# kthohr/mcmc

Measured on AMD Instinct MI355X. Metric: leapfrog-steps/sec (chains*dims*steps/s), HMC d=128 correlated Gaussian, 65536 chains, higher is better.
Workload: dtype f64

## Files before the change

include/mi_mcmc_engine/det_math.hpp:

```cpp
#pragma once

#include <hip/hip_runtime.h>
#include <stdint.h>

#define MI_HD __host__ __device__ __forceinline__

#if defined(__HIP_DEVICE_COMPILE__)
#define MI_NO_DS_MERGE __attribute__((target("no-load-store-opt")))
#else
#define MI_NO_DS_MERGE
#endif

namespace mi {

#ifndef MI_KC_MODE
#define MI_KC_MODE 1
#endif
#if defined(__HIP_DEVICE_COMPILE__) && MI_KC_MODE == 1
__device__ __forceinline__ double mi_kc(double c) { asm volatile("" : "+s"(c)); return c; }
#define MI_KC(c) ::mi::mi_kc(c)
#define MI_KCD(c, dep) ::mi::mi_kc(c)
#elif defined(__HIP_DEVICE_COMPILE__) && MI_KC_MODE == 2
template <uint64_t BITS>
__device__ __forceinline__ double mi_kc()
{
    uint32_t lo, hi;
    asm volatile("s_mov_b32 %0, %2\n\ts_mov_b32 %1, %3" : "=s"(lo), "=s"(hi) : "n"((uint32_t)BITS), "n"((uint32_t)(BITS >> 32)));
    return __builtin_bit_cast(double, ((uint64_t)hi << 32) | (uint64_t)lo);
}
template <uint64_t BITS>
__device__ __forceinline__ double mi_kcd(double dep)
{
    uint32_t lo, hi;
    asm volatile("s_mov_b32 %0, %2\n\ts_mov_b32 %1, %3" : "=s"(lo), "=s"(hi) : "n"((uint32_t)BITS), "n"((uint32_t)(BITS >> 32)), "v"(dep));
    return __builtin_bit_cast(double, ((uint64_t)hi << 32) | (uint64_t)lo);
}
#define MI_KC(c) (::mi::mi_kc<__builtin_bit_cast(uint64_t, (double)(c))>())
#define MI_KCD(c, dep) (::mi::mi_kcd<__builtin_bit_cast(uint64_t, (double)(c))>(dep))
#else
#define MI_KC(c) (c)
#define MI_KCD(c, dep) (c)
#endif


MI_HD uint64_t d2u(double x) { return __builtin_bit_cast(uint64_t, x); }
MI_HD double u2d(uint64_t u) { return __builtin_bit_cast(double, u); }
MI_HD double pow2i(int k) { return u2d((uint64_t)(k + 1023) << 52); }
MI_HD double dfma(double a, double b, double c) { return __builtin_fma(a, b, c); }
MI_HD bool is_finite(double x) { return (d2u(x) & 0x7ff0000000000000ULL) != 0x7ff0000000000000ULL; }

constexpr double LN2_HI = 0x1.62e42fee00000p-1;
constexpr double LN2_LO = 0x1.a39ef35793c76p-33;
constexpr double INV_LN2 = 0x1.71547652b82fep+0;
constexpr double PI_4 = 0x1.921fb54442d18p-1;
constexpr double INF = __builtin_huge_val();

MI_HD double det_exp(double x)
{
    if (x != x) return x;
    if (x > 709.782712893384) return INF;
    if (x < -745.2) return 0.0;
    const double kf = __builtin_rint(x * INV_LN2);
    const int k = (int)kf;
    double r = dfma(-kf, LN2_HI, x);
    r = dfma(-kf, LN2_LO, r);
    double p = MI_KCD(1.0 / 87178291200.0, r);
    p = dfma(p, r, MI_KCD(1.0 / 6227020800.0, p));
    p = dfma(p, r, MI_KCD(1.0 / 479001600.0, p));
    p = dfma(p, r, MI_KCD(1.0 / 39916800.0, p));
    p = dfma(p, r, MI_KCD(1.0 / 3628800.0, p));
    p = dfma(p, r, MI_KCD(1.0 / 362880.0, p));
    p = dfma(p, r, MI_KCD(1.0 / 40320.0, p));
    p = dfma(p, r, MI_KCD(1.0 / 5040.0, p));
    p = dfma(p, r, MI_KCD(1.0 / 720.0, p));
    p = dfma(p, r, MI_KCD(1.0 / 120.0, p));
    p = dfma(p, r, MI_KCD(1.0 / 24.0, p));
    p = dfma(p, r, MI_KCD(1.0 / 6.0, p));
    p = dfma(p, r, 0.5);
    p = dfma(p, r, 1.0);
    p = dfma(p, r, 1.0);
    const int k1 = k / 2, k2 = k - k1;
    return (p * pow2i(k1)) * pow2i(k2);
}

MI_HD double det_log(double x)
{
    if (x != x) return x;
    if (x < 0.0) return __builtin_nan("");
    if (x == 0.0) return -INF;
    if (x == INF) return x;
    int e = 0;
    uint64_t u = d2u(x);
    if ((u >> 52) == 0) { x = x * 0x1p54; u = d2u(x); e = -54; }
    e += (int)(u >> 52) - 1023;
    u = (u & 0x000fffffffffffffULL) | 0x3ff0000000000000ULL;
    double m = u2d(u);
    if (m > 0x1.6a09e667f3bcdp+0) { m = m * 0.5; e += 1; }
    const double f = m - 1.0;
    const double s = f / (2.0 + f);
    const double z = s * s;
    double p = MI_KCD(1.0 / 23.0, z);
    p = dfma(p, z, MI_KCD(1.0 / 21.0, p));
    p = dfma(p, z, MI_KCD(1.0 / 19.0, p));
    p = dfma(p, z, MI_KCD(1.0 / 17.0, p));
    p = dfma(p, z, MI_KCD(1.0 / 15.0, p));
    p = dfma(p, z, MI_KCD(1.0 / 13.0, p));
    p = dfma(p, z, MI_KCD(1.0 / 11.0, p));
    p = dfma(p, z, MI_KCD(1.0 / 9.0, p));
    p = dfma(p, z, MI_KCD(1.0 / 7.0, p));
    p = dfma(p, z, MI_KCD(1.0 / 5.0, p));
    p = dfma(p, z, MI_KCD(1.0 / 3.0, p));
    p = dfma(p, z, 1.0);
    const double lm = (2.0 * s) * p;
    const double ef = (double)e;
    return dfma(ef, LN2_HI, dfma(ef, LN2_LO, lm));
}

MI_HD double det_pow(double x, double y) { return det_exp(y * det_log(x)); }

MI_HD double norm_ppf(double p)
{
    if (p != p) return p;
    if (p <= 0.0) return -INF;
    if (p >= 1.0) return INF;
    const double q = p - 0.5;
    if (__builtin_fabs(q) <= 0.425) {
        const double r = 0.180625 - q * q;
        const double num = (((((((2.5090809287301226727e+3 * r + 3.3430575583588128105e+4) * r + 6.7265770927008700853e+4) * r + 4.5921953931549871457e+4) * r +
                               1.3731693765509461125e+4) * r + 1.9715909503065514427e+3) * r + 1.3314166789178437745e+2) * r + 3.3871328727963666080e+0) * q;
        const double den = (((((((5.2264952788528545610e+3 * r + 2.8729085735721942674e+4) * r + 3.9307895800092710610e+4) * r + 2.1213794301586595867e+4) * r +
                               5.3941960214247511077e+3) * r + 6.8718700749205790830e+2) * r + 4.2313330701600911252e+1) * r + 1.0);
        return num / den;
    }
    double r = __builtin_sqrt(-det_log(q <= 0.0 ? p : 1.0 - p));
    double num, den;
    if (r <= 5.0) {
        r = r - 1.6;
        num = (((((((7.74545014278341407640e-4 * r + 2.27238449892691845833e-2) * r + 2.41780725177450611770e-1) * r + 1.27045825245236838258e+0) * r +
                  3.64784832476320460504e+0) * r + 5.76949722146069140550e+0) * r + 4.63033784615654529590e+0) * r + 1.42343711074968357734e+0);
        den = (((((((1.05075007164441684324e-9 * r + 5.47593808499534494600e-4) * r + 1.51986665636164571966e-2) * r + 1.48103976427480074590e-1) * r +
                  6.89767334985100004550e-1) * r + 1.67638483018380384940e+0) * r + 2.05319162663775882187e+0) * r + 1.0);
    } else {
        r = r - 5.0;
        num = (((((((2.01033439929228813265e-7 * r + 2.71155556874348757815e-5) * r + 1.24266094738807843860e-3) * r + 2.65321895265761230930e-2) * r +
                  2.96560571828504891230e-1) * r + 1.78482653991729133580e+0) * r + 5.46378491116411436990e+0) * r + 6.65790464350110377720e+0);
        den = (((((((2.04426310338993978564e-15 * r + 1.42151175831644588870e-7) * r + 1.84631831751005468180e-5) * r + 7.86869131145613259100e-4) * r +
                  1.48753612908506148525e-2) * r + 1.36929880922735805310e-1) * r + 5.99832206555887937690e-1) * r + 1.0);
    }
    const double x = num / den;
    return q < 0.0 ? -x : x;
}

MI_HD void sincos_kernel(double a, double& s, double& c)
{
    const double z = a * a;
    double ps = MI_KCD(-1.0 / 121645100408832000.0, z);
    ps = dfma(ps, z, MI_KCD(1.0 / 355687428096000.0, ps));
    ps = dfma(ps, z, MI_KCD(-1.0 / 1307674368000.0, ps));
    ps = dfma(ps, z, MI_KCD(1.0 / 6227020800.0, ps));
    ps = dfma(ps, z, MI_KCD(-1.0 / 39916800.0, ps));
    ps = dfma(ps, z, MI_KCD(1.0 / 362880.0, ps));
    ps = dfma(ps, z, MI_KCD(-1.0 / 5040.0, ps));
    ps = dfma(ps, z, MI_KCD(1.0 / 120.0, ps));
    ps = dfma(ps, z, MI_KCD(-1.0 / 6.0, ps));
    ps = dfma(ps, z, 1.0);
    s = a * ps;
    double pc = MI_KCD(1.0 / 6402373705728000.0, z);
    pc = dfma(pc, z, MI_KCD(-1.0 / 20922789888000.0, pc));
    pc = dfma(pc, z, MI_KCD(1.0 / 87178291200.0, pc));
    pc = dfma(pc, z, MI_KCD(-1.0 / 479001600.0, pc));
    pc = dfma(pc, z, MI_KCD(1.0 / 3628800.0, pc));
    pc = dfma(pc, z, MI_KCD(-1.0 / 40320.0, pc));
    pc = dfma(pc, z, MI_KCD(1.0 / 720.0, pc));
    pc = dfma(pc, z, MI_KCD(-1.0 / 24.0, pc));
    pc = dfma(pc, z, 0.5);
    c = dfma(-pc, z, 1.0);
}

MI_HD void det_sincos2pi(double u, double& sn, double& cs)
{
    const double v = u * 8.0;
    const double qf = __builtin_floor(v);
    const int q = (int)qf & 7;
    double t = v - qf;
    if (q & 1) t = 1.0 - t;
    double s, c;
    sincos_kernel(t * PI_4, s, c);
    const bool swap = ((q + 1) & 2) != 0;
    const double cc = swap ? s : c;
    const double ss = swap ? c : s;
    const bool neg_c = (q >= 2) && (q <= 5);
    const bool neg_s = (q >= 4);
    cs = neg_c ? -cc : cc;
    sn = neg_s ? -ss : ss;
}

MI_HD double softplus(double eta)
{
    if (eta > 0.0) return eta + det_log(1.0 + det_exp(-eta));
    return det_log(1.0 + det_exp(eta));
}
MI_HD double sigmoid(double eta)
{
    if (eta >= 0.0) return 1.0 / (1.0 + det_exp(-eta));
    const double e = det_exp(eta);
    return e / (1.0 + e);
}

struct u32x4 { uint32_t x, y, z, w; };

MI_HD uint32_t mulhi32(uint32_t a, uint32_t b) { return (uint32_t)(((uint64_t)a * b) >> 32); }

MI_HD u32x4 philox4x32_10(u32x4 c, uint32_t k0, uint32_t k1)
{
#pragma unroll
    for (int r = 0; r < 10; ++r) {
        const uint64_t p0 = (uint64_t)0xD2511F53u * c.x, p1 = (uint64_t)0xCD9E8D57u * c.z;
        c = u32x4{(uint32_t)(p1 >> 32) ^ c.y ^ k0, (uint32_t)p1, (uint32_t)(p0 >> 32) ^ c.w ^ k1, (uint32_t)p0};
        k0 += 0x9E3779B9u;
        k1 += 0xBB67AE85u;
    }
    return c;
}

MI_HD double u01(uint32_t lo, uint32_t hi)
{
    const uint64_t k = (((uint64_t)hi << 32) | lo) >> 12;
    return (double)(2 * k + 1) * 0x1p-53;
}

enum : uint32_t { STREAM_NORMAL = 0u, STREAM_UNIFORM = 1u, STREAM_INIT = 2u,
                  STREAM_DE_INIT = 3u, STREAM_DE = 4u,
                  STREAM_AEES_NORMAL = 5u, STREAM_AEES = 6u,
                  STREAM_BRIDGE = 7u,
                  STREAM_PREDICT = 8u };

MI_HD u32x4 rng_block(uint64_t seed, uint64_t chain, uint32_t draw, uint32_t slot, uint32_t stream)
{
    const u32x4 c{(uint32_t)chain, draw, slot, stream | ((uint32_t)(chain >> 32) << 8)};
    return philox4x32_10(c, (uint32_t)seed, (uint32_t)(seed >> 32));
}

MI_HD double rng_uniform(uint64_t seed, uint64_t chain, uint32_t draw, uint32_t slot)
{
    const u32x4 w = rng_block(seed, chain, draw, slot, STREAM_UNIFORM);
    return u01(w.x, w.y);
}

MI_HD void rng_normal_pair_core(uint64_t seed, uint64_t chain, uint32_t draw, uint32_t slot, uint32_t stream, double& z0, double& z1)
{
    const u32x4 w = rng_block(seed, chain, draw, slot, stream);
    const double u1 = u01(w.x, w.y);
    const double u2 = u01(w.z, w.w);
    const double r = __builtin_sqrt(-2.0 * det_log(u1));
    double s, c;
    det_sincos2pi(u2, s, c);
    z0 = r * c;
    z1 = r * s;
}
#ifdef MI_RNG_NOINLINE
__attribute__((noinline))
#endif
MI_HD void rng_normal_pair(uint64_t seed, uint64_t chain, uint32_t draw, uint32_t slot, uint32_t stream,
                           double& z0, double& z1)
{
#if defined(__HIP_DEVICE_COMPILE__)
    asm volatile("" : "+v"(slot));
#endif
    rng_normal_pair_core(seed, chain, draw, slot, stream, z0, z1);
}

typedef double rng_double4 __attribute__((ext_vector_type(4)));
__device__ __attribute__((noinline)) inline rng_double4 rng_normal_two_pairs(uint64_t seed, uint64_t chain, uint32_t draw, uint32_t slot_a,
                                                                             uint32_t slot_b, uint32_t stream)
{
#if defined(__HIP_DEVICE_COMPILE__)
    asm volatile("" : "+v"(slot_a), "+v"(slot_b));
#endif
    double a0, a1, b0, b1;
    rng_normal_pair_core(seed, chain, draw, slot_a, stream, a0, a1);
    rng_normal_pair_core(seed, chain, draw, slot_b, stream, b0, b1);
    return rng_double4{a0, a1, b0, b1};
}
typedef double rng_double8 __attribute__((ext_vector_type(8)));
__device__ __attribute__((noinline)) inline rng_double8 rng_normal_four_pairs(uint64_t seed, uint64_t chain, uint32_t draw, uint32_t slot_a,
                                                                              uint32_t slot_step, uint32_t stream)
{
#if defined(__HIP_DEVICE_COMPILE__)
    asm volatile("" : "+v"(slot_a));
#endif
    double z[8];
#pragma unroll
    for (int k = 0; k < 4; ++k) rng_normal_pair_core(seed, chain, draw, slot_a + (uint32_t)k * slot_step, stream, z[2 * k], z[2 * k + 1]);
    return rng_double8{z[0], z[1], z[2], z[3], z[4], z[5], z[6], z[7]};
}

MI_HD void rng_normal_pair_at(uint64_t seed, uint64_t chain, uint32_t draw, uint32_t base, uint32_t j, uint32_t stream,
                              double& z0, double& z1)
{
#if defined(__HIP_DEVICE_COMPILE__)
    asm volatile("" : "+v"(j));
#endif
    rng_normal_pair(seed, chain, draw, base + j, stream, z0, z1);
}


}
```

include/mi_mcmc_engine/hmc_dense.hpp:

```cpp
#pragma once

#include "det_math.hpp"

#ifndef MI_HMC_RNG_STAGED
#define MI_HMC_RNG_STAGED 0
#endif

#ifndef MI_HMC_RNG_PAIRS
#define MI_HMC_RNG_PAIRS 1
#endif

#ifndef MI_HMC_WPB
#define MI_HMC_WPB 8
#endif

namespace mi {

typedef double double4_t __attribute__((ext_vector_type(4)));

struct HmcParams {
    const double* P;
    uint32_t d;
    uint64_t C;
    uint64_t chain0;
    double* theta;
    double* wsave;
    int vals_bound;
    uint32_t draw0;
    const double* Minv;
    const double* Lchol;
    double* draws;
    uint64_t* n_accept;
    uint64_t* n_leap;
    uint64_t seed;
    uint32_t n_burnin, n_keep, n_leap_steps;
    double eps;
    const int* btype;
    const double* lb;
    const double* ub;
    const double* m_sqrt;
    const double* m_inv;
    uint32_t ablate;
    uint32_t stagger;
    uint32_t m_per_chain;
    uint32_t* nf_flag;
    uint32_t sep_target;
};

template <int NS>
__device__ __forceinline__ double dot4(const double (&x)[NS], const double (&y)[NS])
{
    double q = 0.0;
#pragma unroll
    for (int s = 0; s < NS; ++s) q = dfma(x[s], y[s], q);
    q = q + __shfl_xor(q, 32);
    q = q + __shfl_xor(q, 16);
    return q;
}

template <int NS>
__device__ __forceinline__ void dense_product_poison(const double (&x)[NS], double (&y)[NS], int j, uint32_t d)
{
    int nloc = 0;
#pragma unroll
    for (int s = 0; s < NS; ++s) nloc += is_finite(x[s]) ? 0 : 1;
    int n = nloc + __shfl_xor(nloc, 16);
    n = n + __shfl_xor(n, 32);
    if (__ballot(n != 0) == 0ull) return;
#pragma unroll
    for (int s = 0; s < NS; ++s) {
        const int others = n - (is_finite(x[s]) ? 0 : 1);
        if (others > 0 && (uint32_t)(4 * s + j) < d) y[s] = __builtin_nan("");
    }
}

template <int NT>
__device__ __forceinline__ void matvec_mfma(const double* __restrict__ afrag, const double (&th)[4 * NT],
                                            double (&w)[4 * NT])
{
    constexpr int NS = 4 * NT;
    double4_t acc[NT];
    double a_cur[NT], a_nxt[NT];
    typedef const double __attribute__((address_space(3)))* lds_cptr;
    lds_cptr lo = (lds_cptr)afrag;
    uint32_t hi_off = (uint32_t)(uintptr_t)lo + (NT > 4 ? 4u * NS * 64u * 8u : 0u);
    if constexpr (NT > 4) asm volatile("" : "+v"(hi_off));
    lds_cptr hi = (lds_cptr)(uintptr_t)hi_off;
    auto frag = [&](int t, int s) __attribute__((always_inline)) -> double {
        return (NT > 4 && t >= 4) ? hi[((t - 4) * NS + s) * 64] : lo[(t * NS + s) * 64];
    };
#pragma unroll
    for (int t = 0; t < NT; ++t) {
        acc[t] = double4_t{0.0, 0.0, 0.0, 0.0};
        a_cur[t] = frag(t, 0);
    }
#pragma unroll
    for (int s = 0; s < NS; ++s) {
        if (s + 1 < NS) {
#pragma unroll
            for (int t = 0; t < NT; ++t) a_nxt[t] = frag(t, s + 1);
        }
        __builtin_amdgcn_sched_barrier(0);
#pragma unroll
        for (int t = 0; t < NT; ++t)
            acc[t] = __builtin_amdgcn_mfma_f64_16x16x4f64(a_cur[t], th[s], acc[t], 0, 0, 0);
        __builtin_amdgcn_sched_barrier(0);
#pragma unroll
        for (int t = 0; t < NT; ++t) a_cur[t] = a_nxt[t];
    }
#pragma unroll
    for (int t = 0; t < NT; ++t) {
        w[4 * t + 0] = acc[t][0];
        w[4 * t + 1] = acc[t][1];
        w[4 * t + 2] = acc[t][2];
        w[4 * t + 3] = acc[t][3];
    }
}

template <int NT>
__device__ __forceinline__ void stage_precision(const double* __restrict__ P, uint32_t d, double* lds)
{
    constexpr int NS = 4 * NT;
    const int lane = threadIdx.x & 63, wave = threadIdx.x >> 6, nw = blockDim.x >> 6;
    for (int f = wave; f < NT * NS; f += nw) {
        const int t = f / NS, s = f % NS;
        const uint32_t row = 16 * t + (lane & 15), col = 4 * s + (lane >> 4);
        lds[f * 64 + lane] = (row < d && col < d) ? P[(size_t)row * d + col] : 0.0;
    }
    __syncthreads();
}


template <int NT>
__device__ __forceinline__ void matvec_mfma_g(const double* __restrict__ gfrag, const double (&th)[4 * NT], double (&w)[4 * NT])
{
    constexpr int NS = 4 * NT;
    constexpr int PD = 3;
    uint32_t b_lo = (uint32_t)__builtin_amdgcn_readfirstlane((int)(uint32_t)(uintptr_t)gfrag);
    uint32_t b_hi = (uint32_t)__builtin_amdgcn_readfirstlane((int)(uint32_t)((uintptr_t)gfrag >> 32));
    asm volatile("" : "+s"(b_lo), "+s"(b_hi));
    const double* const gbase = reinterpret_cast<const double*>(((uintptr_t)b_hi << 32) | (uintptr_t)b_lo);
    const uint32_t lane_ = (uint32_t)(threadIdx.x & 63);
    auto frag = [&](int t, int s_) -> double { return gbase[(uint32_t)((t * NS + s_) * 64) + lane_]; };
    double4_t acc[NT];
    double a[PD + 1][NT];
#pragma unroll
    for (int t = 0; t < NT; ++t) acc[t] = double4_t{0.0, 0.0, 0.0, 0.0};
#pragma unroll
    for (int p = 0; p < PD && p < NS; ++p)
#pragma unroll
        for (int t = 0; t < NT; ++t) a[p][t] = frag(t, p);
#pragma unroll
    for (int s = 0; s < NS; ++s) {
        if (s + PD < NS) {
#pragma unroll
            for (int t = 0; t < NT; ++t) a[(s + PD) % (PD + 1)][t] = frag(t, s + PD);
        }
        __builtin_amdgcn_sched_barrier(0);
#pragma unroll
        for (int t = 0; t < NT; ++t)
            acc[t] = __builtin_amdgcn_mfma_f64_16x16x4f64(a[s % (PD + 1)][t], th[s], acc[t], 0, 0, 0);
        __builtin_amdgcn_sched_barrier(0);
    }
#pragma unroll
    for (int t = 0; t < NT; ++t) {
        w[4 * t + 0] = acc[t][0];
        w[4 * t + 1] = acc[t][1];
        w[4 * t + 2] = acc[t][2];
        w[4 * t + 3] = acc[t][3];
    }
}

template <int NT>
constexpr bool dense_m_from_global() { return NT > 4; }
template <int NT>
__device__ __forceinline__ void matvec_m2(const double* __restrict__ frag_lane, const double (&x)[4 * NT], double (&y)[4 * NT])
{
    if constexpr (dense_m_from_global<NT>()) matvec_mfma_g<NT>(frag_lane, x, y);
    else matvec_mfma<NT>(frag_lane, x, y);
}

template <int NT>
__device__ __forceinline__ void target_times(const double* __restrict__ afrag, const double* __restrict__ P, uint32_t d, bool sep,
                                             const double (&x)[4 * NT], double (&w)[4 * NT])
{
    if (sep) {
        const uint32_t j = (threadIdx.x & 63u) >> 4;
#pragma unroll
        for (int s = 0; s < 4 * NT; ++s) {
            const uint32_t dim = 4u * (uint32_t)s + j;
            w[s] = (dim < d) ? P[(size_t)dim * (d + 1u)] * x[s] : 0.0;
        }
    } else matvec_mfma<NT>(afrag, x, w);
}

constexpr double EPS_DBL = 2.220446049250313e-16;

#define MI_BOX_INLINE __attribute__((noinline))
__device__ MI_BOX_INLINE double box_transform(double v, int bt, double lb, double ub)
{
    switch (bt) {
    case 2: return det_log(v - lb + EPS_DBL);
    case 3: return -det_log(ub - v + EPS_DBL);
    case 4: return det_log(v - lb + EPS_DBL) - det_log(ub - v + EPS_DBL);
    default: return v;
    }
}
__device__ MI_BOX_INLINE double box_inv_transform(double v, int bt, double lb, double ub)
{
    switch (bt) {
    case 2: return !is_finite(v) ? lb + EPS_DBL : lb + EPS_DBL + det_exp(v);
    case 3: return !is_finite(v) ? ub - EPS_DBL : ub - EPS_DBL - det_exp(-v);
    case 4: {
        if (!is_finite(v)) {
            if (v != v) return (ub - lb) / 2;
            return (v < 0.0) ? lb + EPS_DBL : ub - EPS_DBL;
        }
        const double e = det_exp(v);
        const double r = (lb - EPS_DBL + (ub + EPS_DBL) * e) / (1.0 + e);
        return is_finite(r) ? r : ub - EPS_DBL;
    }
    default: return v;
    }
}
__device__ MI_BOX_INLINE double box_inv_jacobian(double v, int bt, double lb, double ub)
{
    switch (bt) {
    case 2: return det_exp(-v);
    case 3: return det_exp(v);
    case 4: { const double e = det_exp(v); return ((e + 1) * (e + 1)) / (e * (ub - lb)); }
    default: return 1.0;
    }
}
__device__ MI_BOX_INLINE double box_log_jacobian_term(double v, int bt, double lb, double ub)
{
    switch (bt) {
    case 2: return v;
    case 3: return -v;
    case 4: {
        const double e = det_exp(v);
        if (is_finite(e)) return det_log(ub - lb) + v - 2 * det_log(1 + e);
        return det_log(ub - lb) - v;
    }
    default: return 0.0;
    }
}

template <int NT, int WPB, bool BOUNDED = false, bool DENSE_M = false, bool DIAGM = false, bool PCM = false>
__global__ MI_NO_DS_MERGE __launch_bounds__(64 * WPB, WPB / 4) void hmc_gauss_mfma_kernel(const HmcParams prm)
{
    static_assert(!PCM || DIAGM, "per-chain masses ride the diagonal-mass variant");
    static_assert(!DENSE_M || BOUNDED, "the dense preconditioner rides the general variant");
    static_assert(!DIAGM || !BOUNDED, "DIAGM is the plain kernel with a diagonal mass; bounds take the general variant");
    constexpr int NS = 4 * NT;
    extern __shared__ __attribute__((aligned(16))) double lds_P[];
    stage_precision<NT>(prm.P, prm.d, lds_P);
    double* lds_lb = lds_P + NT * NS * 64;
    double* lds_ub = lds_lb + 16 * NT;
    double* lds_ms = lds_ub + 16 * NT;
    double* lds_mi = lds_ms + 16 * NT;
    int* lds_bt = reinterpret_cast<int*>(lds_mi + 16 * NT);
    double* lds_Minv = lds_mi + 16 * NT + 8 * NT;
    double* lds_L = lds_Minv + NT * NS * 64;
    if constexpr (DENSE_M && !dense_m_from_global<NT>()) {
        stage_precision<NT>(prm.Minv, prm.d, lds_Minv);
        stage_precision<NT>(prm.Lchol, prm.d, lds_L);
    }
    if (BOUNDED) {
        for (int i = threadIdx.x; i < 16 * NT; i += blockDim.x) {
            const bool in = (uint32_t)i < prm.d;
            lds_lb[i] = in ? prm.lb[i] : 0.0;
            lds_ub[i] = in ? prm.ub[i] : 0.0;
            lds_bt[i] = in ? prm.btype[i] : 1;
            lds_ms[i] = in ? prm.m_sqrt[i] : 1.0;
            lds_mi[i] = in ? prm.m_inv[i] : 1.0;
        }
        __syncthreads();
    }
    if (DIAGM && !PCM) {
        for (int i = threadIdx.x; i < 16 * NT; i += blockDim.x) {
            const bool in = (uint32_t)i < prm.d;
            lds_ms[i] = in ? prm.m_sqrt[i] : 1.0;
            lds_mi[i] = in ? prm.m_inv[i] : 1.0;
        }
        __syncthreads();
    }

    const int lane = threadIdx.x & 63, wave = threadIdx.x >> 6;
    const int j = lane >> 4;
    uint32_t bslices = 0;
    if constexpr (BOUNDED) {
        if (prm.vals_bound)
            for (int s_ = 0; s_ < 4 * NT; ++s_) {
                const bool any = lds_bt[4 * s_] != 1 || lds_bt[4 * s_ + 1] != 1 || lds_bt[4 * s_ + 2] != 1 || lds_bt[4 * s_ + 3] != 1;
                bslices |= (any ? 1u : 0u) << s_;
            }
        bslices = (uint32_t)__builtin_amdgcn_readfirstlane((int)bslices);
    }
    auto slice_bounded = [&](int s) -> bool { return ((bslices >> s) & 1u) != 0u; };
    [[maybe_unused]] auto mi_col = [&]() __attribute__((always_inline)) -> const double* {
        const double* p = lds_mi + (lane >> 4);
        asm volatile("" : "+v"(p));
        return p;
    };
    const uint64_t cl = ((uint64_t)blockIdx.x * WPB + wave) * 16 + (lane & 15);
    const bool live = cl < prm.C;
    const uint64_t cld = live ? cl : prm.C - 1;
    [[maybe_unused]] auto pcm_at = [&](const double* tab, int s) __attribute__((always_inline)) -> double {
        uint32_t dim = 4u * (uint32_t)s + (uint32_t)(lane >> 4);
        asm volatile("" : "+v"(dim));
        return tab[(size_t)(dim < prm.d ? dim : 0u) * prm.C + cld];
    };
    auto minv_at = [&]([[maybe_unused]] const double* mic, int s) __attribute__((always_inline)) -> double {
        if constexpr (PCM) return pcm_at(prm.m_inv, s); else return mic[4 * s];
    };
    const uint64_t chain = prm.chain0 + cl;
    const uint32_t d = prm.d;
    const uint64_t C = prm.C;
    const double eps = prm.eps;
    const double* afrag = lds_P + lane;
    [[maybe_unused]] const double* afrag_minv = (DENSE_M && dense_m_from_global<NT>()) ? prm.Minv + lane : lds_Minv + lane;
    [[maybe_unused]] const double* afrag_l = (DENSE_M && dense_m_from_global<NT>()) ? prm.Lchol + lane : lds_L + lane;

    double th[NS], pm[NS], w[NS];
    double xs[BOUNDED ? NS : 1];
    const size_t lane_off = (size_t)j * C + cld;
    double* const ws_wave = prm.wsave + ((size_t)blockIdx.x * WPB + wave) * ((size_t)3 * NS * 64) + lane;
    auto ws_group = [&](int k) -> double* {
        double* b = ws_wave + (size_t)(k & ~7) * 64;
        asm volatile("" : "+v"(b));
        return b + (k & 7) * 64;
    };
    auto th_mem = [&](int s) -> double* { return ws_group(s); };
    auto w_mem = [&](int s) -> double* { return ws_group(NS + s); };
    [[maybe_unused]] auto z_mem = [&](int s) -> double* { return ws_wave + (size_t)(2 * NS + s) * 64; };

    auto gradient = [&]() __attribute__((always_inline)) {
        if constexpr (BOUNDED) {
#pragma unroll
            for (int s = 0; s < NS; ++s) {
                const int i = 4 * s + j;
                if (slice_bounded(s)) xs[s] = ((uint32_t)i < d) ? box_inv_transform(th[s], lds_bt[i], lds_lb[i], lds_ub[i]) : 0.0;
                else xs[s] = ((uint32_t)i < d) ? th[s] : 0.0;
            }
            target_times<NT>(afrag, prm.P, d, prm.sep_target != 0u, xs, w);
        } else {
            matvec_mfma<NT>(afrag, th, w);
        }
    };
    auto kick_terms = [&](double (&t)[BOUNDED ? NS : 1]) __attribute__((always_inline)) {
        if constexpr (BOUNDED) {
#pragma unroll
            for (int s = 0; s < NS; ++s) {
                const int i = 4 * s + j;
                if (slice_bounded(s)) t[s] = box_inv_jacobian(th[s], lds_bt[i], lds_lb[i], lds_ub[i]) * w[s];
                else t[s] = 1.0 * w[s];
            }
            if (prm.vals_bound) dense_product_poison<NS>(w, t, j, d);
#pragma unroll
            for (int s = 0; s < NS; ++s) t[s] = (eps * t[s]) / 2.0;
        }
    };
    auto kinetic = [&]() __attribute__((always_inline)) -> double {
        if constexpr (BOUNDED) {
            double mp[NS];
            if constexpr (DENSE_M) {
                matvec_m2<NT>(afrag_minv, pm, mp);
            } else {
#pragma unroll
                for (int s = 0; s < NS; ++s) mp[s] = lds_mi[4 * s + j] * pm[s];
                dense_product_poison<NS>(pm, mp, j, d);
            }
            double q = 0.0;
#pragma unroll
            for (int s = 0; s < NS; ++s) q = dfma(pm[s], mp[s], q);
            q = q + __shfl_xor(q, 32);
            q = q + __shfl_xor(q, 16);
            return q / 2.0;
        } else if constexpr (DIAGM) {
            double q = 0.0;
            const double* mic = PCM ? nullptr : mi_col();
#pragma unroll
            for (int s = 0; s < NS; ++s) q = dfma(pm[s], minv_at(mic, s) * pm[s], q);
            q = q + __shfl_xor(q, 32);
            q = q + __shfl_xor(q, 16);
            return q / 2.0;
        } else {
            return dot4<NS>(pm, pm) / 2.0;
        }
    };
    auto potential = [&]() __attribute__((always_inline)) -> double {
        if constexpr (BOUNDED) {
            const double kval = -0.5 * dot4<NS>(xs, w);
            double lj = 0.0;
#pragma unroll
            for (int s = 0; s < NS; ++s) {
                if (!slice_bounded(s)) continue;
                const int i0 = 4 * s;
                const int bt = lds_bt[4 * s + j];
                const double term = box_log_jacobian_term(th[s], bt, lds_lb[4 * s + j], lds_ub[4 * s + j]);
#pragma unroll
                for (int g = 0; g < 4; ++g) {
                    const double tg = __shfl(term, (lane & 15) + 16 * g);
                    if ((uint32_t)(i0 + g) < d && lds_bt[i0 + g] != 1) lj = lj + tg;
                }
            }
            return -(kval + lj);
        } else {
            return 0.5 * dot4<NS>(th, w);
        }
    };

#pragma unroll
    for (int s = 0; s < NS; ++s) {
        const uint32_t dim = 4 * s + j;
        const double v = prm.theta[(size_t)(dim < d ? dim : 0u) * C + cld];
        if constexpr (BOUNDED) th[s] = (dim < d) ? box_transform(v, lds_bt[dim], lds_lb[dim], lds_ub[dim]) : 0.0;
        else th[s] = (dim < d) ? v : 0.0;
    }
    gradient();
    if (live) {
#pragma unroll
        for (int s = 0; s < NS; ++s) { *th_mem(s) = th[s]; *w_mem(s) = w[s]; }
    }
    double prev_U = potential();
    uint64_t n_acc = 0;
    const uint32_t n_total = prm.n_burnin + prm.n_keep;
    [[maybe_unused]] bool nf_seen = false;

    if (WPB > 4 && wave >= 4)
        for (uint32_t k = 0; k < prm.stagger; ++k) __builtin_amdgcn_s_sleep(127);

    const unsigned long long t_loop0 = clock64();
#pragma unroll 1
    for (uint32_t draw = 0; draw < n_total; ++draw) {
#if MI_HMC_RNG_STAGED
#pragma unroll 1
        for (int b = 0; b < NS / 2; ++b) {
            double z0, z1;
            if (prm.ablate & 4u) { z0 = 0.25; z1 = -0.5; }
            else rng_normal_pair_at(prm.seed, chain, draw + prm.draw0, (uint32_t)(4 * b), (uint32_t)j, STREAM_NORMAL, z0, z1);
            *z_mem(2 * b) = (8u * b + j < d) ? z0 : 0.0;
            *z_mem(2 * b + 1) = (8u * b + 4 + j < d) ? z1 : 0.0;
        }
#pragma unroll
        for (int s = 0; s < NS; ++s) pm[s] = *z_mem(s);
        if constexpr (DENSE_M) {
            double zz[NS];
#pragma unroll
            for (int s = 0; s < NS; ++s) zz[s] = pm[s];
            matvec_m2<NT>(afrag_l, zz, pm);
        } else if constexpr (BOUNDED || DIAGM) {
#pragma unroll
            for (int s = 0; s < NS; ++s) pm[s] = lds_ms[4 * s + j] * pm[s];
        }
#else
#pragma unroll
        for (int b = 0; b < NS / 2; ++b) {
            double z0, z1;
            if (prm.ablate & 4u) { z0 = 0.25; z1 = -0.5; }
            else rng_normal_pair_at(prm.seed, chain, draw + prm.draw0, (uint32_t)(4 * b), (uint32_t)j, STREAM_NORMAL, z0, z1);
            pm[2 * b] = (8u * b + j < d) ? z0 : 0.0;
            pm[2 * b + 1] = (8u * b + 4 + j < d) ? z1 : 0.0;
            if constexpr (DIAGM && PCM) {
                pm[2 * b] = pcm_at(prm.m_sqrt, 2 * b) * pm[2 * b];
                pm[2 * b + 1] = pcm_at(prm.m_sqrt, 2 * b + 1) * pm[2 * b + 1];
            } else if constexpr (DIAGM) {
                const double* msc = lds_ms + (lane >> 4);
                asm volatile("" : "+v"(msc));
                pm[2 * b] = msc[8 * b] * pm[2 * b];
                pm[2 * b + 1] = msc[8 * b + 4] * pm[2 * b + 1];
            } else if constexpr (BOUNDED && !DENSE_M) {
                pm[2 * b] = lds_ms[8 * b + j] * pm[2 * b];
                pm[2 * b + 1] = lds_ms[8 * b + 4 + j] * pm[2 * b + 1];
            }
            if (BOUNDED || MI_HMC_RNG_PAIRS == 1 || (b & 1)) __builtin_amdgcn_sched_barrier(0);
        }
        if constexpr (DENSE_M) {
            double zz[NS];
#pragma unroll
            for (int s = 0; s < NS; ++s) zz[s] = pm[s];
            matvec_m2<NT>(afrag_l, zz, pm);
        }
#endif
        const double prev_K = kinetic();

        if constexpr (!BOUNDED) {
            const uint32_t L = prm.n_leap_steps;
            if (L > 0 && (prm.ablate & 3u) != 1u) {
                [[maybe_unused]] const double* mic = (DIAGM && !PCM) ? mi_col() : nullptr;
#pragma unroll
                for (int s = 0; s < NS; ++s) {
                    pm[s] = pm[s] - (eps * w[s]) / 2.0;
                    if constexpr (DIAGM) th[s] = th[s] + eps * (minv_at(mic, s) * pm[s]);
                    else th[s] = th[s] + eps * pm[s];
                }
            }
#pragma unroll 1
            for (uint32_t k = 0; k + 1 < L; ++k) {
                if ((prm.ablate & 3u) != 2u) gradient();
                if ((prm.ablate & 3u) != 1u) {
                    [[maybe_unused]] const double* mic = (DIAGM && !PCM) ? mi_col() : nullptr;
#pragma unroll
                    for (int s = 0; s < NS; ++s) {
                        const double t = (eps * w[s]) / 2.0;
                        pm[s] = pm[s] - t;
                        pm[s] = pm[s] - t;
                        if constexpr (DIAGM) th[s] = th[s] + eps * (minv_at(mic, s) * pm[s]);
                        else th[s] = th[s] + eps * pm[s];
                    }
                }
            }
            if (L > 0) {
                if ((prm.ablate & 3u) != 2u) gradient();
                if ((prm.ablate & 3u) != 1u) {
#pragma unroll
                    for (int s = 0; s < NS; ++s) pm[s] = pm[s] - (eps * w[s]) / 2.0;
                }
            }
        } else {
            const uint32_t L = prm.n_leap_steps;
            auto drift_step = [&]() __attribute__((always_inline)) {
                double mp[NS];
                if constexpr (DENSE_M) {
                    matvec_m2<NT>(afrag_minv, pm, mp);
                } else {
#pragma unroll
                    for (int s = 0; s < NS; ++s) mp[s] = lds_mi[4 * s + j] * pm[s];
                    dense_product_poison<NS>(pm, mp, j, d);
                }
#pragma unroll
                for (int s = 0; s < NS; ++s) th[s] = th[s] + eps * mp[s];
            };
            if (L > 0) {
                double t[NS];
                kick_terms(t);
#pragma unroll
                for (int s = 0; s < NS; ++s) pm[s] = pm[s] - t[s];
                drift_step();
            }
#pragma unroll 1
            for (uint32_t k = 0; k + 1 < L; ++k) {
                gradient();
                double t[NS];
                kick_terms(t);
#pragma unroll
                for (int s = 0; s < NS; ++s) {
                    pm[s] = pm[s] - t[s];
                    pm[s] = pm[s] - t[s];
                }
                drift_step();
            }
            if (L > 0) {
                gradient();
                double t[NS];
                kick_terms(t);
#pragma unroll
                for (int s = 0; s < NS; ++s) pm[s] = pm[s] - t[s];
            }
        }
        if constexpr (BOUNDED) { if (prm.n_leap_steps == 0) gradient(); }

        double prop_U = potential();
        const bool u_nf = !is_finite(prop_U);
        if (u_nf) prop_U = INF;
        const double prop_K = kinetic();
        if constexpr (!BOUNDED) nf_seen |= u_nf | !is_finite(prop_K);
        const double x = -(prop_U + prop_K) + (prev_U + prev_K);
        const double comp_val = (x < 0.01) ? x : 0.01;
        const double z = rng_uniform(prm.seed, chain, draw + prm.draw0, 0u);
        const bool accept = z < det_exp(comp_val);
#ifndef MI_HMC_NO_WSAVE
#define MI_HMC_NO_WSAVE 0
#endif
        if constexpr (MI_HMC_NO_WSAVE && !BOUNDED) {
            if (accept) {
                prev_U = prop_U;
                if (live && !(prm.ablate & 8u)) {
#pragma unroll
                    for (int s = 0; s < NS; ++s) *th_mem(s) = th[s];
                }
            }
            if (__ballot(!accept) != 0ull) {
                if (!accept) {
#pragma unroll
                    for (int s = 0; s < NS; ++s) th[s] = *th_mem(s);
                }
                gradient();
            }
        } else
        if (accept) {
            prev_U = prop_U;
            if (live && !(prm.ablate & 8u)) {
#pragma unroll
                for (int s = 0; s < NS; ++s) { *th_mem(s) = th[s]; *w_mem(s) = w[s]; }
            }
        } else {
#pragma unroll
            for (int s = 0; s < NS; ++s) { th[s] = *th_mem(s); w[s] = *w_mem(s); }
        }
        if (draw >= prm.n_burnin) {
            n_acc += accept ? 1u : 0u;
            if (prm.draws != nullptr && live && !(prm.ablate & 16u)) {
                double* out = prm.draws + (size_t)(draw - prm.n_burnin) * d * C;
#pragma unroll
                for (int s = 0; s < NS; ++s) {
                    const uint32_t dim = 4 * s + j;
                    if (dim < d) (out + (size_t)(4 * s) * C)[lane_off] =
                        (BOUNDED && slice_bounded(s)) ? box_inv_transform(th[s], lds_bt[dim], lds_lb[dim], lds_ub[dim]) : th[s];
                }
            }
        }
    }

    bool replay = false;
    if constexpr (!BOUNDED) replay = nf_seen && prm.nf_flag != nullptr;
    if (live && replay && j == 0) { prm.nf_flag[cl] = 1u; prm.nf_flag[C] = 1u; }
    if (live && !replay) {
#pragma unroll
        for (int s = 0; s < NS; ++s) {
            const uint32_t dim = 4 * s + j;
            if (dim < d) prm.theta[(size_t)dim * C + cl] =
                (BOUNDED && slice_bounded(s)) ? box_inv_transform(th[s], lds_bt[dim], lds_lb[dim], lds_ub[dim]) : th[s];
        }
    }
    if (live && !replay && j == 0) {
        if (prm.n_accept) prm.n_accept[cl] = n_acc;
        if (prm.n_leap) prm.n_leap[cl] = (prm.ablate & 32u) ? (uint64_t)(clock64() - t_loop0)
                                                            : (uint64_t)n_total * prm.n_leap_steps;
    }
}

}
```

mcmc_amd/csrc/hmc_launch.hip:

```cpp
#include "hmc_dense.hpp"
#include "hmc_split.hpp"
#include "launchers.hpp"
#include "launch_common.hpp"

namespace mi {
namespace {

template <int NT>
int plain(const HmcParams& prm, hipStream_t st)
{
    constexpr int WPB = MI_HMC_WPB;
    const size_t lds = (size_t)NT * 4 * NT * 64 * sizeof(double);
    auto kern = hmc_gauss_mfma_kernel<NT, WPB>;
    MI_LAUNCH_TRY(hipFuncSetAttribute(reinterpret_cast<const void*>(kern), hipFuncAttributeMaxDynamicSharedMemorySize, (int)lds));
    const unsigned grid = (unsigned)((prm.C + 16 * WPB - 1) / (16 * WPB));
    note_kernel("hmc_gauss_mfma_kernel<%d, %d, false, false, false>", NT, WPB);
    hipLaunchKernelGGL(kern, dim3(grid), dim3(64 * WPB), lds, st, prm);
    return (int)hipGetLastError();
}

template <int NT, bool PCM = false>
int plain_diagm(const HmcParams& prm, hipStream_t st)
{
    constexpr int WPB = MI_HMC_WPB;
    const size_t lds = (size_t)NT * 4 * NT * 64 * sizeof(double) + (size_t)16 * NT * (4 * sizeof(double) + sizeof(int));
    auto kern = hmc_gauss_mfma_kernel<NT, WPB, false, false, true, PCM>;
    MI_LAUNCH_TRY(hipFuncSetAttribute(reinterpret_cast<const void*>(kern), hipFuncAttributeMaxDynamicSharedMemorySize, (int)lds));
    const unsigned grid = (unsigned)((prm.C + 16 * WPB - 1) / (16 * WPB));
    note_kernel("hmc_gauss_mfma_kernel<%d, %d, false, false, true%s>", NT, WPB, PCM ? ", true" : "");
    hipLaunchKernelGGL(kern, dim3(grid), dim3(64 * WPB), lds, st, prm);
    return (int)hipGetLastError();
}

template <int NT>
int plain4(const HmcParams& prm, hipStream_t st)
{
    const size_t lds = (size_t)NT * 4 * NT * 64 * sizeof(double);
    auto kern = hmc_gauss_mfma_kernel<NT, 4>;
    MI_LAUNCH_TRY(hipFuncSetAttribute(reinterpret_cast<const void*>(kern), hipFuncAttributeMaxDynamicSharedMemorySize, (int)lds));
    note_kernel("hmc_gauss_mfma_kernel<%d, 4, false, false, false>", NT);
    hipLaunchKernelGGL(kern, dim3((unsigned)((prm.C + 63) / 64)), dim3(256), lds, st, prm);
    return (int)hipGetLastError();
}

template <int NT, int SPLIT, int WPB>
int split(const HmcParams& prm, hipStream_t st)
{
    const size_t lds = hmc_split_lds_bytes<NT, SPLIT, WPB>();
    int dev = 0, lds_max = 0;
    MI_LAUNCH_TRY(hipGetDevice(&dev));
    MI_LAUNCH_TRY(hipDeviceGetAttribute(&lds_max, hipDeviceAttributeMaxSharedMemoryPerBlock, dev));
    if ((size_t)lds_max < lds) return (int)hipErrorInvalidValue;
    auto kern = hmc_gauss_split_kernel<NT, SPLIT, WPB>;
    MI_LAUNCH_TRY(hipFuncSetAttribute(reinterpret_cast<const void*>(kern), hipFuncAttributeMaxDynamicSharedMemorySize, (int)lds));
    const unsigned chains_per_wg = 16 * (WPB / SPLIT);
    note_kernel("hmc_gauss_split_kernel<%d, %d, %d>", NT, SPLIT, WPB);
    hipLaunchKernelGGL(kern, dim3((unsigned)((prm.C + chains_per_wg - 1) / chains_per_wg)), dim3(64 * WPB), lds, st, prm);
    return (int)hipGetLastError();
}

}

int launch_hmc_gauss(const HmcParams& prm, int nt, bool gen, bool dense_m, hipStream_t st)
{
    if (dense_m) return launch_hmc_gauss_dense_m(prm, nt, st);
    if (gen) return launch_hmc_gauss_general(prm, nt, st);
    return MI_DISPATCH_NT(nt, plain<1>(prm, st), plain<2>(prm, st), plain<4>(prm, st), plain<8>(prm, st));
}

int launch_hmc_gauss_diagm(const HmcParams& prm, int nt, hipStream_t st)
{
    if (prm.m_per_chain)
        return MI_DISPATCH_NT(nt, (plain_diagm<1, true>(prm, st)), (plain_diagm<2, true>(prm, st)), (plain_diagm<4, true>(prm, st)), (plain_diagm<8, true>(prm, st)));
    return MI_DISPATCH_NT(nt, plain_diagm<1>(prm, st), plain_diagm<2>(prm, st), plain_diagm<4>(prm, st), plain_diagm<8>(prm, st));
}

int launch_hmc_gauss_few_chains(const HmcParams& prm, int shape, hipStream_t st)
{
    return shape == 1 ? plain4<8>(prm, st) : shape == 2 ? split<8, 2, 4>(prm, st) : shape == 3 ? split<8, 4, 8>(prm, st) : split<8, 4, 4>(prm, st);
}

}
```

Before: 267.1 billion.

## Add full-tile HMC kernel variant with scalar-base global addressing and bitop3 Philox

Adds a FULL_TILE specialization of the plain HMC kernel, used when d equals the tile size and C is small enough. It fixes d at compile time, which drops the bounds checks. Workspace and draw/theta stores use SGPR base pointers plus a 32-bit per-lane offset, so 64-bit VGPR address arithmetic goes away. The accept/reject save and restore gets an explicit schedule barrier, and the variant adds manual vmcnt waits. Separately, Philox's three-way XORs now use the gfx950 bitop3 instruction, which cuts VALU work in RNG generation.

```diff
diff --git a/include/mi_mcmc_engine/det_math.hpp b/include/mi_mcmc_engine/det_math.hpp
--- a/include/mi_mcmc_engine/det_math.hpp
+++ b/include/mi_mcmc_engine/det_math.hpp
@@ -211,12 +211,21 @@
 
 MI_HD uint32_t mulhi32(uint32_t a, uint32_t b) { return (uint32_t)(((uint64_t)a * b) >> 32); }
 
+MI_HD uint32_t xor3(uint32_t a, uint32_t b, uint32_t c)
+{
+#if defined(__HIP_DEVICE_COMPILE__) && defined(__gfx950__) && __has_builtin(__builtin_amdgcn_bitop3_b32)
+    return __builtin_amdgcn_bitop3_b32(a, b, c, 0x96);
+#else
+    return a ^ b ^ c;
+#endif
+}
+
 MI_HD u32x4 philox4x32_10(u32x4 c, uint32_t k0, uint32_t k1)
 {
 #pragma unroll
     for (int r = 0; r < 10; ++r) {
         const uint64_t p0 = (uint64_t)0xD2511F53u * c.x, p1 = (uint64_t)0xCD9E8D57u * c.z;
-        c = u32x4{(uint32_t)(p1 >> 32) ^ c.y ^ k0, (uint32_t)p1, (uint32_t)(p0 >> 32) ^ c.w ^ k1, (uint32_t)p0};
+        c = u32x4{xor3((uint32_t)(p1 >> 32), c.y, k0), (uint32_t)p1, xor3((uint32_t)(p0 >> 32), c.w, k1), (uint32_t)p0};
         k0 += 0x9E3779B9u;
         k1 += 0xBB67AE85u;
     }
diff --git a/include/mi_mcmc_engine/hmc_dense.hpp b/include/mi_mcmc_engine/hmc_dense.hpp
--- a/include/mi_mcmc_engine/hmc_dense.hpp
+++ b/include/mi_mcmc_engine/hmc_dense.hpp
@@ -246,15 +246,16 @@
     }
 }
 
-template <int NT, int WPB, bool BOUNDED = false, bool DENSE_M = false, bool DIAGM = false, bool PCM = false>
+template <int NT, int WPB, bool BOUNDED = false, bool DENSE_M = false, bool DIAGM = false, bool PCM = false, bool FULL_TILE = false>
 __global__ MI_NO_DS_MERGE __launch_bounds__(64 * WPB, WPB / 4) void hmc_gauss_mfma_kernel(const HmcParams prm)
 {
     static_assert(!PCM || DIAGM, "per-chain masses ride the diagonal-mass variant");
     static_assert(!DENSE_M || BOUNDED, "the dense preconditioner rides the general variant");
     static_assert(!DIAGM || !BOUNDED, "DIAGM is the plain kernel with a diagonal mass; bounds take the general variant");
+    static_assert(!FULL_TILE || (!BOUNDED && !DIAGM), "the full-tile path is the plain kernel's");
     constexpr int NS = 4 * NT;
     extern __shared__ __attribute__((aligned(16))) double lds_P[];
-    stage_precision<NT>(prm.P, prm.d, lds_P);
+    stage_precision<NT>(prm.P, FULL_TILE ? 16u * NT : prm.d, lds_P);
     double* lds_lb = lds_P + NT * NS * 64;
     double* lds_ub = lds_lb + 16 * NT;
     double* lds_ms = lds_ub + 16 * NT;
@@ -315,7 +316,7 @@
         if constexpr (PCM) return pcm_at(prm.m_inv, s); else return mic[4 * s];
     };
     const uint64_t chain = prm.chain0 + cl;
-    const uint32_t d = prm.d;
+    const uint32_t d = FULL_TILE ? 16u * NT : prm.d;
     const uint64_t C = prm.C;
     const double eps = prm.eps;
     const double* afrag = lds_P + lane;
@@ -331,8 +332,29 @@
         asm volatile("" : "+v"(b));
         return b + (k & 7) * 64;
     };
-    auto th_mem = [&](int s) -> double* { return ws_group(s); };
-    auto w_mem = [&](int s) -> double* { return ws_group(NS + s); };
+    typedef double __attribute__((address_space(1)))* gbl_dptr;
+    typedef char __attribute__((address_space(1)))* gbl_bptr;
+    [[maybe_unused]] const uintptr_t ws_u = (uintptr_t)prm.wsave
+        + ((size_t)blockIdx.x * WPB + (size_t)__builtin_amdgcn_readfirstlane(wave)) * ((size_t)3 * NS * 64 * sizeof(double));
+    [[maybe_unused]] uint32_t ws_lane = (uint32_t)lane * 8u;
+    [[maybe_unused]] auto ws_group_u = [&](int k) __attribute__((always_inline)) -> gbl_dptr {
+        uintptr_t b = ws_u + (uintptr_t)(k & ~7) * 512u;
+        asm volatile("" : "+s"(b));
+        return (gbl_dptr)((gbl_bptr)b + ws_lane + (k & 7) * 512);
+    };
+    [[maybe_unused]] uint32_t row_lane = (uint32_t)(lane_off * sizeof(double));
+    [[maybe_unused]] auto store_row_u = [&](double* row0) __attribute__((always_inline)) {
+        uintptr_t rb = (uintptr_t)row0;
+#pragma unroll
+        for (int s = 0; s < NS; ++s) {
+            asm volatile("" : "+s"(rb));
+            *(gbl_dptr)((gbl_bptr)rb + row_lane) = th[s];
+            rb += (uintptr_t)(4 * sizeof(double)) * C;
+        }
+    };
+    [[maybe_unused]] auto vmem_settled = [&]() __attribute__((always_inline)) { __builtin_amdgcn_s_waitcnt(0x0F70); };
+    auto th_mem = [&](int s) __attribute__((always_inline)) { if constexpr (FULL_TILE) return ws_group_u(s); else return ws_group(s); };
+    auto w_mem = [&](int s) __attribute__((always_inline)) { if constexpr (FULL_TILE) return ws_group_u(NS + s); else return ws_group(NS + s); };
     [[maybe_unused]] auto z_mem = [&](int s) -> double* { return ws_wave + (size_t)(2 * NS + s) * 64; };
 
     auto gradient = [&]() __attribute__((always_inline)) {
@@ -434,6 +456,7 @@
     const unsigned long long t_loop0 = clock64();
 #pragma unroll 1
     for (uint32_t draw = 0; draw < n_total; ++draw) {
+        if constexpr (FULL_TILE) asm volatile("" : "+v"(ws_lane), "+v"(row_lane));
 #if MI_HMC_RNG_STAGED
 #pragma unroll 1
         for (int b = 0; b < NS / 2; ++b) {
@@ -483,6 +506,7 @@
             matvec_m2<NT>(afrag_l, zz, pm);
         }
 #endif
+        if constexpr (FULL_TILE) vmem_settled();
         const double prev_K = kinetic();
 
         if constexpr (!BOUNDED) {
@@ -588,6 +612,19 @@
                 }
                 gradient();
             }
+        } else if constexpr (FULL_TILE) {
+            if (accept) {
+                prev_U = prop_U;
+                if (live && !(prm.ablate & 8u)) {
+#pragma unroll
+                    for (int s = 0; s < NS; ++s) { *th_mem(s) = th[s]; *w_mem(s) = w[s]; }
+                }
+            }
+            __builtin_amdgcn_sched_barrier(0);
+            if (!accept) {
+#pragma unroll
+                for (int s = 0; s < NS; ++s) { th[s] = *th_mem(s); w[s] = *w_mem(s); }
+            }
         } else
         if (accept) {
             prev_U = prop_U;
@@ -603,11 +640,14 @@
             n_acc += accept ? 1u : 0u;
             if (prm.draws != nullptr && live && !(prm.ablate & 16u)) {
                 double* out = prm.draws + (size_t)(draw - prm.n_burnin) * d * C;
-#pragma unroll
-                for (int s = 0; s < NS; ++s) {
-                    const uint32_t dim = 4 * s + j;
-                    if (dim < d) (out + (size_t)(4 * s) * C)[lane_off] =
-                        (BOUNDED && slice_bounded(s)) ? box_inv_transform(th[s], lds_bt[dim], lds_lb[dim], lds_ub[dim]) : th[s];
+                if constexpr (FULL_TILE) { vmem_settled(); store_row_u(out); }
+                else {
+#pragma unroll
+                    for (int s = 0; s < NS; ++s) {
+                        const uint32_t dim = 4 * s + j;
+                        if (dim < d) (out + (size_t)(4 * s) * C)[lane_off] =
+                            (BOUNDED && slice_bounded(s)) ? box_inv_transform(th[s], lds_bt[dim], lds_lb[dim], lds_ub[dim]) : th[s];
+                    }
                 }
             }
         }
@@ -617,11 +657,14 @@
     if constexpr (!BOUNDED) replay = nf_seen && prm.nf_flag != nullptr;
     if (live && replay && j == 0) { prm.nf_flag[cl] = 1u; prm.nf_flag[C] = 1u; }
     if (live && !replay) {
-#pragma unroll
-        for (int s = 0; s < NS; ++s) {
-            const uint32_t dim = 4 * s + j;
-            if (dim < d) prm.theta[(size_t)dim * C + cl] =
-                (BOUNDED && slice_bounded(s)) ? box_inv_transform(th[s], lds_bt[dim], lds_lb[dim], lds_ub[dim]) : th[s];
+        if constexpr (FULL_TILE) store_row_u(prm.theta);
+        else {
+#pragma unroll
+            for (int s = 0; s < NS; ++s) {
+                const uint32_t dim = 4 * s + j;
+                if (dim < d) prm.theta[(size_t)dim * C + cl] =
+                    (BOUNDED && slice_bounded(s)) ? box_inv_transform(th[s], lds_bt[dim], lds_lb[dim], lds_ub[dim]) : th[s];
+            }
         }
     }
     if (live && !replay && j == 0) {
diff --git a/mcmc_amd/csrc/hmc_launch.hip b/mcmc_amd/csrc/hmc_launch.hip
--- a/mcmc_amd/csrc/hmc_launch.hip
+++ b/mcmc_amd/csrc/hmc_launch.hip
@@ -6,12 +6,19 @@
 namespace mi {
 namespace {
 
+template <int NT, int WPB>
+auto plain_kernel(const HmcParams& prm)
+{
+    const bool full = prm.d == 16u * NT && prm.C < (1ull << 27);
+    return full ? hmc_gauss_mfma_kernel<NT, WPB, false, false, false, false, true> : hmc_gauss_mfma_kernel<NT, WPB>;
+}
+
 template <int NT>
 int plain(const HmcParams& prm, hipStream_t st)
 {
     constexpr int WPB = MI_HMC_WPB;
     const size_t lds = (size_t)NT * 4 * NT * 64 * sizeof(double);
-    auto kern = hmc_gauss_mfma_kernel<NT, WPB>;
+    auto kern = plain_kernel<NT, WPB>(prm);
     MI_LAUNCH_TRY(hipFuncSetAttribute(reinterpret_cast<const void*>(kern), hipFuncAttributeMaxDynamicSharedMemorySize, (int)lds));
     const unsigned grid = (unsigned)((prm.C + 16 * WPB - 1) / (16 * WPB));
     note_kernel("hmc_gauss_mfma_kernel<%d, %d, false, false, false>", NT, WPB);
@@ -36,7 +43,7 @@
 int plain4(const HmcParams& prm, hipStream_t st)
 {
     const size_t lds = (size_t)NT * 4 * NT * 64 * sizeof(double);
-    auto kern = hmc_gauss_mfma_kernel<NT, 4>;
+    auto kern = plain_kernel<NT, 4>(prm);
     MI_LAUNCH_TRY(hipFuncSetAttribute(reinterpret_cast<const void*>(kern), hipFuncAttributeMaxDynamicSharedMemorySize, (int)lds));
     note_kernel("hmc_gauss_mfma_kernel<%d, 4, false, false, false>", NT);
     hipLaunchKernelGGL(kern, dim3((unsigned)((prm.C + 63) / 64)), dim3(256), lds, st, prm);
```

Measured after the change: 270.3 billion, median of 6. 1.2% higher.
